# peteroh23/ModulationDetectionCNN

Hardware: AMD Instinct MI355X
Metric: I/Q frames/sec (2x128, VT-CNN2, batch=2^20) (higher is better)
Workload: dtype bf16; 1 GPU; vtcnn2-c11-bf16-n2^20; topology=vtcnn2, classes=11, frames_per_gpu=1048576, global_batch=1048576, parallelism=batch-shard x1 (no collective), outputs=softmax probabilities f32 + argmax int32, frames_per_forward_call=1048576, full=False

## Files before the change

### modulationdetectioncnn_amd/csrc/vtcnn2_bf16_sched.hip

```cpp
#include "vtcnn2_bf16_common.h"
#include "vtcnn2_sched_common.h"

#include <cmath>
#include <cstdlib>
#include <type_traits>

namespace mdc {

namespace {

constexpr int kNV = 24;

struct SchedState {
    u32x4 Wv[kNV];
    u32x4 Wa[kWFrags - kNV];
    f32x4 bias[5];
    u32x4 A1[2];
    unsigned Bf[2][2][2][4];
    f32x16 X[2];
    f32x4 rp[4];
    float rc[4];
    float tprev;
    u32x4 L0[3];
    u32x4 L1;
    unsigned cb[4];
    unsigned wr_addr, rd_addr, rc_addr, im_addr;
    int gs;
};

template <int SP, int J, int I, bool PAD = false>
__device__ __forceinline__ void sch_tap(SchedState& st, f32x4 (&acc)[5]) {
    constexpr int CT = 1 - I / 10, BB = (I / 5) % 2, OT = I % 5;
    constexpr int IDX = ((CT * 3 + J) * 2 + BB) * 5 + OT;
    const u32x4 b = u32x4{st.Bf[SP][CT][BB][0], st.Bf[SP][CT][BB][1], st.Bf[SP][CT][BB][2], st.Bf[SP][CT][BB][3]};
    if constexpr (J == 0 && I < 5) {
        if constexpr (IDX < kNV) asm volatile("v_mfma_f32_16x16x32_bf16 %0, %1, %2, %3" : "=&a"(acc[OT]) : "v"(st.Wv[IDX]), "v"(b), "a"(st.bias[OT]));
        else asm volatile("v_mfma_f32_16x16x32_bf16 %0, %1, %2, %3" : "=&a"(acc[OT]) : "a"(st.Wa[IDX - kNV]), "v"(b), "a"(st.bias[OT]));
    } else if constexpr (PAD) {
        static_assert(IDX >= kNV, "padded form written for the AGPR-resident fragments only");
        asm volatile("s_nop 1\n\tv_mfma_f32_16x16x32_bf16 %0, %1, %2, %0" : "+a"(acc[OT]) : "a"(st.Wa[IDX - kNV]), "v"(b));
    } else {
        if constexpr (IDX < kNV) asm volatile("v_mfma_f32_16x16x32_bf16 %0, %1, %2, %0" : "+a"(acc[OT]) : "v"(st.Wv[IDX]), "v"(b));
        else asm volatile("v_mfma_f32_16x16x32_bf16 %0, %1, %2, %0" : "+a"(acc[OT]) : "a"(st.Wa[IDX - kNV]), "v"(b));
    }
}
template <int SP, int U>
__device__ __forceinline__ void sch_packop(SchedState& st) {
    constexpr int CT = U >> 3, j = U & 7;
    unsigned& d = st.Bf[SP][CT][j >> 2][j & 3];
    const float lo = st.X[CT][2 * j], hi = st.X[CT][2 * j + 1];
    asm volatile("v_cvt_pk_bf16_f32 %0, %1, %2 clamp" : "=v"(d) : "v"(lo), "v"(hi));
}
template <int V12, bool FIRST, bool LAST, int ABL, bool RANGE = false>
__device__ __forceinline__ void sch_step(SchedState& st, int v, int q, unsigned short* fbase, f32x4 (&acc)[3][5], int wlo = 0) {
    constexpr int PAR = V12 & 1, PN = 1 - PAR;
    constexpr int R1 = (V12 + 1) & 3, S0 = ((V12 + 1) >> 2) % 3, SN = (S0 + 1) % 3;
    constexpr bool kLoadEven = (V12 & 3) == 1 && !LAST, kLoadOdd = (V12 & 3) == 3 && !LAST;
    constexpr int LSLOT = ((V12 >> 2) + 1) % 3;
    constexpr bool kExch = ABL != 2 && ABL != 6, kFin = ABL != 3 && ABL != 6, kC1 = ABL != 5 && ABL != 6;
    f32x4 (&a2)[5] = acc[V12 % 3];
    f32x4 (&a1)[5] = acc[(V12 + 1) % 3];
    f32x4 (&a0)[5] = acc[(V12 + 2) % 3];
    const unsigned load_addr = st.im_addr + ((v >> 2) * 16 + (kLoadEven ? 16 : 24));
    FinTmp ft;
    FinOut fo;
    constexpr int OP = (V12 + 1) & 1;
#define FIN(K) do { if (!FIRST && kFin) sch_fin_clamp<K, OP>(st, ft, fo); } while (0)
#define PREP(I) do { if (!LAST && kC1 && ABL != 11) sch_prep<R1, S0, SN, I>(st); } while (0)
#define C1M(CT) do { if (!LAST && kC1) sch_conv1_mfma<R1, S0, CT>(st); } while (0)
#define ST(W) do { if (!FIRST && kFin && (W == 0 || OP == 1)) { if (ABL == 7) { if (W == 0) asm volatile("" ::"v"(fo.o0), "v"(fo.o1)); else asm volatile("" ::"v"(fo.tt)); } else if (!RANGE || v - 1 >= wlo) sch_store<W>(fo, fbase, v - 1, q, st.gs); } } while (0)
#define WR(OT) do { if (kExch && ABL != 8) sch_part_write<PAR, OT>(st, a2[OT]); } while (0)
#define PK(N) do { if (!LAST && kC1 && ABL != 10) sch_packop<PN, N>(st); } while (0)
#define RD(R) do { if (kExch && ABL != 9) sch_red_load1<PAR, R>(st); } while (0)
#define LD() do { if (kC1 && ABL != 11) { if (kLoadEven) sch_load_even<LSLOT>(st, load_addr); else if (kLoadOdd) sch_load_odd(st, load_addr); } } while (0)
#ifdef MDC_F8_PROBE_HALF_BARRIER
    constexpr bool kHalfBarrierSkip = (V12 & 1) == 1;
#else
    constexpr bool kHalfBarrierSkip = false;
#endif
#define HANDOFF() do { \
        if (ABL == 1 || kHalfBarrierSkip) asm volatile("s_waitcnt lgkmcnt(0)" ::: "memory"); \
        else if (kExch) asm volatile("s_waitcnt lgkmcnt(0)\n\ts_barrier" ::: "memory"); \
        asm volatile("" ::"a"(a2[0]), "a"(a2[1]), "a"(a2[2]), "a"(a2[3]), "a"(a2[4])); } while (0)
    sch_wait_lds(st);
    sch_tap<PAR, 2, 0, RANGE && (V12 == 1 || V12 == 2)>(st, a2); FIN(0);
    sch_tap<PAR, 2, 1>(st, a2); FIN(1);
    sch_tap<PAR, 2, 2>(st, a2); FIN(2);
    sch_tap<PAR, 2, 3>(st, a2); FIN(3);
    sch_tap<PAR, 2, 4>(st, a2); FIN(4);
    sch_tap<PAR, 2, 5>(st, a2); FIN(5);
    sch_tap<PAR, 2, 6>(st, a2); FIN(6);
    sch_tap<PAR, 2, 7>(st, a2); FIN(7);
    sch_tap<PAR, 2, 8>(st, a2); FIN(8);
    sch_tap<PAR, 2, 9>(st, a2); FIN(9);
    sch_tap<PAR, 2, 10>(st, a2); FIN(10);
    sch_tap<PAR, 2, 11>(st, a2); FIN(11);
    sch_tap<PAR, 2, 12>(st, a2); FIN(12);
    sch_tap<PAR, 2, 13>(st, a2); FIN(13);
    sch_tap<PAR, 2, 14>(st, a2); FIN(14);
    sch_tap<PAR, 2, 15>(st, a2); FIN(15);
    sch_tap<PAR, 2, 16>(st, a2); PREP(0);
    sch_tap<PAR, 2, 17>(st, a2); PREP(1);
    sch_tap<PAR, 2, 18>(st, a2); PREP(2);
    sch_tap<PAR, 2, 19>(st, a2); PREP(3);
    C1M(0); WR(0); FIN(16); FIN(17);
    C1M(1); WR(1);
    sch_tap<PAR, 1, 0>(st, a1); ST(0);
    sch_tap<PAR, 1, 1>(st, a1); WR(2);
    sch_tap<PAR, 1, 2>(st, a1); ST(1);
    sch_tap<PAR, 1, 3>(st, a1); PK(0);
    sch_tap<PAR, 1, 4>(st, a1); WR(3);
    sch_tap<PAR, 1, 5>(st, a1); PK(1);
    sch_tap<PAR, 1, 6>(st, a1); PK(2);
    sch_tap<PAR, 1, 7>(st, a1); WR(4);
    sch_tap<PAR, 1, 8>(st, a1); PK(3);
    sch_tap<PAR, 1, 9>(st, a1); PK(4);
    sch_tap<PAR, 1, 10>(st, a1); PK(5);
    sch_tap<PAR, 1, 11>(st, a1); PK(6);
    sch_tap<PAR, 1, 12>(st, a1); PK(7);
    sch_tap<PAR, 1, 13>(st, a1); PK(8);
    sch_tap<PAR, 1, 14>(st, a1); PK(9);
    sch_tap<PAR, 1, 15>(st, a1); PK(10);
    sch_tap<PAR, 1, 16>(st, a1); PK(11);
    sch_tap<PAR, 1, 17>(st, a1); PK(12);
    sch_tap<PAR, 1, 18>(st, a1); PK(13);
    sch_tap<PAR, 1, 19>(st, a1); PK(14);
    sch_tap<PAR, 0, 0>(st, a0); PK(15);
    sch_tap<PAR, 0, 1>(st, a0);
    sch_tap<PAR, 0, 2>(st, a0);
    sch_tap<PAR, 0, 3>(st, a0);
    sch_tap<PAR, 0, 4>(st, a0);
    sch_tap<PAR, 0, 5>(st, a0);
    sch_tap<PAR, 0, 6>(st, a0); HANDOFF();
    sch_tap<PAR, 0, 7>(st, a0); RD(0);
    sch_tap<PAR, 0, 8>(st, a0); RD(1);
    sch_tap<PAR, 0, 9>(st, a0); RD(2);
    sch_tap<PAR, 0, 10>(st, a0); RD(3);
    sch_tap<PAR, 0, 11>(st, a0); RD(4);
    sch_tap<PAR, 0, 12>(st, a0); RD(5);
    sch_tap<PAR, 0, 13>(st, a0); RD(6);
    sch_tap<PAR, 0, 14>(st, a0); RD(7);
    sch_tap<PAR, 0, 15>(st, a0); LD();
    sch_tap<PAR, 0, 16>(st, a0);
    sch_tap<PAR, 0, 17>(st, a0);
    sch_tap<PAR, 0, 18>(st, a0);
    sch_tap<PAR, 0, 19>(st, a0);
    if (ABL == 10 && !LAST) asm volatile("" ::"v"(st.X[0]), "v"(st.X[1]));
#undef FIN
#undef PREP
#undef C1M
#undef ST
#undef WR
#undef PK
#undef RD
#undef LD
#undef HANDOFF
}

template <int ABL, bool U8 = false, bool RANGE = false>
__global__ __launch_bounds__(256, 1) void vt_conv_bf16_sched_kernel(const float* __restrict__ x, long n,
                                                                    const u32x4* __restrict__ wq, const u32x4* __restrict__ a1q,
                                                                    const float* __restrict__ b2, unsigned short* __restrict__ feat,
                                                                    long hop2 = 256, float scale = 0.f) {
    extern __shared__ __attribute__((aligned(16))) unsigned char smem[];
    unsigned* img = reinterpret_cast<unsigned*>(smem);
    const int tid = threadIdx.x, lane = tid & 63;
    const int q = __builtin_amdgcn_readfirstlane(tid >> 6);
// ... 17 lines not shown
    const unsigned part_lds = (unsigned)(size_t)(__attribute__((address_space(3))) unsigned char*)(smem + (size_t)2 * kSImgWords * 4);
    const unsigned img_lds = (unsigned)(size_t)(__attribute__((address_space(3))) unsigned char*)smem;
    auto entry = [](int f, int gg) { return 8 * (4 * (f >> 3) + gg) + ((f & 7) ^ (gg >> 1)); };
    const int fs = lane >> 2, gs = lane & 3;
    st.gs = gs;
    st.wr_addr = part_lds + (q * 5 * 64 + entry(nl, g)) * 16;
    st.rd_addr = part_lds + (q * 64 + entry(fs, gs)) * 16;
    st.rc_addr = part_lds + (4 * 64 + entry(fs, q)) * 16 + gs * 4;
#pragma unroll
    for (int k = 0; k < 4; ++k) { st.rp[k] = f32x4{0.f, 0.f, 0.f, 0.f}; st.rc[k] = 0.f; }
#pragma unroll
    for (int s = 0; s < 3; ++s) st.L0[s] = u32x4{0u, 0u, 0u, 0u};
    st.L1 = u32x4{0u, 0u, 0u, 0u};
    st.cb[0] = st.cb[1] = st.cb[2] = st.cb[3] = 0u;
    st.tprev = 0.f;

    for (int i = tid; i < 2 * kSImgWords; i += 256) img[i] = ((((i / kS) & 63) >= 32) && ((i % kS) & 1)) ? 0x3F803F80u : 0u;
    __syncthreads();
    const long ngroups = (n + 15) >> 4;
    long grp = blockIdx.x;
    if (grp < ngroups)
        for (int k = 0; k < 4; ++k) sch_stage_write(k, stage_decode<U8>(stage_load<U8>(k, x, n, grp * 16, tid, hop2), tid, scale), n, grp * 16, img, tid);
    __syncthreads();
    const int rng = RANGE ? (int)blockIdx.y : 0;
    const int S = 12 * rng;
    const int wlo = rng ? S + 2 : 0;

    int buf = 0;
    for (; grp < ngroups; grp += gridDim.x, buf ^= 1) {
        st.im_addr = img_lds + (buf * kSImgWords + lane * kS) * 4;
        unsigned short* fbase = feat + (grp * 16 + fs) * (long)(kW2 * kC2);
        const long gnext = RANGE ? ngroups : grp + gridDim.x;
        f32x4 acc[3][5];
        {
            const u32x4 zero = u32x4{0u, 0u, 0u, 0u};
#pragma unroll
            for (int b = 0; b < 5; ++b) {
                asm volatile("s_nop 1\n\tv_mfma_f32_16x16x32_bf16 %0, %1, %1, %2" : "=&a"(acc[0][b]) : "v"(zero), "a"(st.bias[b]));
                asm volatile("v_mfma_f32_16x16x32_bf16 %0, %1, %1, %2" : "=&a"(acc[1][b]) : "v"(zero), "a"(st.bias[b]));
            }
        }

        sch_load_even<0>(st, st.im_addr + (S >> 2) * 16);
        sch_load_odd(st, st.im_addr + (S >> 2) * 16 + 8);
        sch_wait_lds(st);
        sch_conv1_mfma<0, 0, 0>(st); sch_conv1_mfma<0, 0, 1>(st);
        asm volatile("s_nop 7\n\ts_nop 7\n\ts_nop 7\n\ts_nop 7\n\ts_nop 7\n\ts_nop 7\n\ts_nop 7\n\ts_nop 7" : "+v"(st.X[0]), "+v"(st.X[1]));
        [&]<int... N>(std::integer_sequence<int, N...>) { (sch_packop<0, N>(st), ...); }(std::make_integer_sequence<int, 16>{});
        asm volatile("s_nop 1");

        sch_step<0, true, false, ABL, RANGE>(st, S, q, fbase, acc, wlo);
        const int iters = RANGE ? (rng < 10 ? 1 : 0) : 10;
        int v = S + 1;
        typename StageRaw<U8>::type sv{};
        for (int it = 0; it < iters; ++it, v += 12) {
            if constexpr (!RANGE) {
                if (it >= 6 && gnext < ngroups) sch_stage_write(it - 6, stage_decode<U8>(sv, tid, scale), n, gnext * 16, img + (buf ^ 1) * kSImgWords, tid);
                if (it >= 5 && it < 9 && gnext < ngroups) sv = stage_load<U8>(it - 5, x, n, gnext * 16, tid, hop2);
            }
            sch_step<1, false, false, ABL, RANGE>(st, v + 0, q, fbase, acc, wlo);
            sch_step<2, false, false, ABL, RANGE>(st, v + 1, q, fbase, acc, wlo);
            sch_step<3, false, false, ABL, RANGE>(st, v + 2, q, fbase, acc, wlo);
            sch_step<4, false, false, ABL, RANGE>(st, v + 3, q, fbase, acc, wlo);
            sch_step<5, false, false, ABL, RANGE>(st, v + 4, q, fbase, acc, wlo);
            sch_step<6, false, false, ABL, RANGE>(st, v + 5, q, fbase, acc, wlo);
            sch_step<7, false, false, ABL, RANGE>(st, v + 6, q, fbase, acc, wlo);
            sch_step<8, false, false, ABL, RANGE>(st, v + 7, q, fbase, acc, wlo);
            sch_step<9, false, false, ABL, RANGE>(st, v + 8, q, fbase, acc, wlo);
            sch_step<10, false, false, ABL, RANGE>(st, v + 9, q, fbase, acc, wlo);
            sch_step<11, false, false, ABL, RANGE>(st, v + 10, q, fbase, acc, wlo);
            sch_step<0, false, false, ABL, RANGE>(st, v + 11, q, fbase, acc, wlo);
        }
        const int vt = RANGE ? v : 121;
        sch_step<1, false, false, ABL, RANGE>(st, vt, q, fbase, acc, wlo);
        if constexpr (RANGE) {
            if (rng < 10) {
                FinOut fo;
                sch_wait_lds(st);
                sch_fin_all_clamp<1>(st, fo);
                sch_store<0>(fo, fbase, vt, q, st.gs);
                sch_store<1>(fo, fbase, vt, q, st.gs);
                asm volatile("s_nop 7\n\ts_nop 7" ::"a"(acc[0][0]), "a"(acc[1][0]), "a"(acc[2][0]));
                __syncthreads();
                continue;
            }
        }
        sch_step<2, false, false, ABL, RANGE>(st, 122, q, fbase, acc, wlo);
        sch_step<3, false, false, ABL, RANGE>(st, 123, q, fbase, acc, wlo);
        sch_step<4, false, false, ABL, RANGE>(st, 124, q, fbase, acc, wlo);
        sch_step<5, false, false, ABL, RANGE>(st, 125, q, fbase, acc, wlo);
        sch_step<6, false, false, ABL, RANGE>(st, 126, q, fbase, acc, wlo);
        sch_step<7, false, false, ABL, RANGE>(st, 127, q, fbase, acc, wlo);
        sch_step<8, false, false, ABL, RANGE>(st, 128, q, fbase, acc, wlo);
        sch_step<9, false, true, ABL, RANGE>(st, 129, q, fbase, acc, wlo);
        auto finish_store = [&](auto odd, int w) {
            FinOut fo;
            sch_wait_lds(st);
            sch_fin_all_clamp<decltype(odd)::value>(st, fo);
            sch_store<0>(fo, fbase, w, q, st.gs);
            if constexpr (decltype(odd)::value) sch_store<1>(fo, fbase, w, q, st.gs);
        };
        using Even = std::integral_constant<int, 0>;
        using Odd = std::integral_constant<int, 1>;
        finish_store(Odd{}, 129);
        asm volatile("s_nop 7\n\ts_nop 7");
        sch_part_write<0, 0>(st, acc[1][0]); sch_part_write<0, 1>(st, acc[1][1]); sch_part_write<0, 2>(st, acc[1][2]);
        sch_part_write<0, 3>(st, acc[1][3]); sch_part_write<0, 4>(st, acc[1][4]);
        asm volatile("s_waitcnt lgkmcnt(0)\n\ts_barrier" ::: "memory");
        sch_red_load<0>(st);
        asm volatile("" ::"a"(acc[1][0]), "a"(acc[1][1]), "a"(acc[1][2]), "a"(acc[1][3]), "a"(acc[1][4]));
        finish_store(Even{}, 130);
        sch_part_write<1, 0>(st, acc[2][0]); sch_part_write<1, 1>(st, acc[2][1]); sch_part_write<1, 2>(st, acc[2][2]);
        sch_part_write<1, 3>(st, acc[2][3]); sch_part_write<1, 4>(st, acc[2][4]);
        asm volatile("s_waitcnt lgkmcnt(0)\n\ts_barrier" ::: "memory");
        sch_red_load<1>(st);
        asm volatile("" ::"a"(acc[2][0]), "a"(acc[2][1]), "a"(acc[2][2]), "a"(acc[2][3]), "a"(acc[2][4]));
        finish_store(Odd{}, 131);
        __syncthreads();
    }
}

}

int vtcnn2_bf16_pack_sched(mdc_model* m) {
    const float* k1 = m->hk[0].data();
    const float* b1 = m->hb[0].data();
    const float* k2 = m->hk[1].data();
    int rc;
    std::vector<unsigned short> wq((size_t)4 * kWFrags * 64 * 8);
    for (int q = 0; q < 4; ++q)
        for (int ct = 0; ct < 2; ++ct)
            for (int j = 0; j < 3; ++j)
                for (int bb = 0; bb < 2; ++bb)
// ... 20 lines not shown
                }
                if (khalf == 0) {
                    d[0] = th[0]; d[1] = th[1]; d[2] = th[0]; d[3] = th[1]; d[4] = th[2]; d[6] = th[2];
                } else {
                    const unsigned short bh = f2bf(b1[ch] * sc);
                    d[0] = tl[0]; d[1] = tl[1]; d[2] = bh; d[3] = f2bf(b1[ch] * sc - bf2f(bh)); d[4] = tl[2];
                }
            }
    return upload(m, 7, a1.data(), a1.size() * 2);
}

int vtcnn2_bf16_conv_sched(const mdc_model* m, const float* x, int64_t n, void* feat, hipStream_t s, long hop2, float scale) {
    const long ngroups = (n + 15) / 16;
    const unsigned grid = (unsigned)(ngroups < 256 ? ngroups : 256);
#define MDC_LAUNCH_SCHED_V(U, R, GRID) do { \
    MDC_HIP(hipFuncSetAttribute(reinterpret_cast<const void*>(vt_conv_bf16_sched_kernel<0, U, R>), hipFuncAttributeMaxDynamicSharedMemorySize, (int)kSchedLds)); \
    hipLaunchKernelGGL((vt_conv_bf16_sched_kernel<0, U, R>), GRID, dim3(256), kSchedLds, s, x, (long)n, \
                       static_cast<const u32x4*>(m->d_pack[6]), static_cast<const u32x4*>(m->d_pack[7]), \
                       static_cast<const float*>(m->d_pack[2]), static_cast<unsigned short*>(feat), hop2 > 0 ? hop2 : 256L, scale); \
    MDC_HIP(hipGetLastError()); return MDC_OK; } while (0)
    if (n <= kConvRangeFrames) {
        if (hop2 > 0) MDC_LAUNCH_SCHED_V(true, true, dim3((unsigned)ngroups, 11));
        else MDC_LAUNCH_SCHED_V(false, true, dim3((unsigned)ngroups, 11));
    }
    if (hop2 > 0) MDC_LAUNCH_SCHED_V(true, false, dim3(grid));
#undef MDC_LAUNCH_SCHED_V
#define MDC_LAUNCH_SCHED(A) do { \
    MDC_HIP(hipFuncSetAttribute(reinterpret_cast<const void*>(vt_conv_bf16_sched_kernel<A>), hipFuncAttributeMaxDynamicSharedMemorySize, (int)kSchedLds)); \
    hipLaunchKernelGGL(vt_conv_bf16_sched_kernel<A>, dim3(grid), dim3(256), kSchedLds, s, x, (long)n, \
                       static_cast<const u32x4*>(m->d_pack[6]), static_cast<const u32x4*>(m->d_pack[7]), \
                       static_cast<const float*>(m->d_pack[2]), static_cast<unsigned short*>(feat), 256L, 0.f); } while (0)
#ifdef MDC_ABLATIONS
    static const int abl = getenv("MDC_ABLATE_S") ? atoi(getenv("MDC_ABLATE_S")) : 0;
    switch (abl) { case 1: MDC_LAUNCH_SCHED(1); break; case 2: MDC_LAUNCH_SCHED(2); break; case 3: MDC_LAUNCH_SCHED(3); break;
                   case 5: MDC_LAUNCH_SCHED(5); break; case 6: MDC_LAUNCH_SCHED(6); break; case 7: MDC_LAUNCH_SCHED(7); break;
                   case 8: MDC_LAUNCH_SCHED(8); break; case 9: MDC_LAUNCH_SCHED(9); break; case 10: MDC_LAUNCH_SCHED(10); break;
                   case 11: MDC_LAUNCH_SCHED(11); break; default: MDC_LAUNCH_SCHED(0); }
#else
    MDC_LAUNCH_SCHED(0);
#endif
#undef MDC_LAUNCH_SCHED
    MDC_HIP(hipGetLastError());
    return MDC_OK;
}

}
```

### modulationdetectioncnn_amd/csrc/vtcnn2_sched_common.h

```cpp
#pragma once
#include "vtcnn2_bf16_common.h"

#include <type_traits>
#include <utility>

namespace mdc {

namespace {

constexpr int kS = 140;
constexpr int kSImgWords = 64 * kS;
constexpr long kConvRangeFrames = 1024;
constexpr size_t kSchedLds = (size_t)2 * kSImgWords * 4 + (size_t)2 * kPartFloats * 4;

using f32x16 = __attribute__((ext_vector_type(16))) float;

template <int SLOT, class S>
__device__ __forceinline__ void sch_load_even(S& st, unsigned entry_addr) {
    asm volatile("ds_read_b128 %0, %1" : "=v"(st.L0[SLOT]) : "v"(entry_addr) : "memory");
}
template <class S>
__device__ __forceinline__ void sch_load_odd(S& st, unsigned entry_addr) {
    asm volatile("ds_read2_b64 %0, %1 offset0:0 offset1:1" : "=v"(st.L1) : "v"(entry_addr) : "memory");
}
// ... 18 lines not shown
template <int PB, int OT, class S>
__device__ __forceinline__ void sch_part_write(S& st, const f32x4& a) {
    asm volatile("ds_write_b128 %0, %1 offset:%2" ::"v"(st.wr_addr), "a"(a), "i"(PB * kPartFloats * 4 + OT * 1024) : "memory");
}
template <int PB, int R, class S>
__device__ __forceinline__ void sch_red_load1(S& st) {
    constexpr int K = R >> 1;
    if constexpr ((R & 1) == 0) asm volatile("ds_read_b128 %0, %1 offset:%2" : "=v"(st.rp[K]) : "v"(st.rd_addr), "i"(PB * kPartFloats * 4 + K * 5120) : "memory");
    else asm volatile("ds_read_b32 %0, %1 offset:%2" : "=v"(st.rc[K]) : "v"(st.rc_addr), "i"(PB * kPartFloats * 4 + K * 5120) : "memory");
}
template <int PB, class S>
__device__ __forceinline__ void sch_red_load(S& st) {
    sch_red_load1<PB, 0>(st); sch_red_load1<PB, 1>(st); sch_red_load1<PB, 2>(st); sch_red_load1<PB, 3>(st);
    sch_red_load1<PB, 4>(st); sch_red_load1<PB, 5>(st); sch_red_load1<PB, 6>(st); sch_red_load1<PB, 7>(st);
}
template <class S>
__device__ __forceinline__ void sch_wait_lds(S& st) {
    asm volatile("s_waitcnt lgkmcnt(0)"
                 : "+v"(st.rp[0]), "+v"(st.rp[1]), "+v"(st.rp[2]), "+v"(st.rp[3]), "+v"(st.rc[0]), "+v"(st.rc[1]), "+v"(st.rc[2]),
                   "+v"(st.rc[3]), "+v"(st.L0[0]), "+v"(st.L0[1]), "+v"(st.L0[2]), "+v"(st.L1)
                 :: "memory");
}
struct FinOut { unsigned o0, o1, tt; };
struct FinTmp { float s[4], u[4], a, b, t; };
constexpr int kFeatShift = 32;

template <int K, int ODD, class S>
__device__ __forceinline__ void sch_fin_clamp(S& st, FinTmp& f, FinOut& out) {
    if constexpr (K < 4) asm volatile("v_add_f32 %0, %1, %2" : "=v"(f.s[K]) : "v"(st.rp[0][K]), "v"(st.rp[1][K]));
    else if constexpr (K < 8) asm volatile("v_add_f32 %0, %1, %2" : "=v"(f.u[K - 4]) : "v"(st.rp[2][K - 4]), "v"(st.rp[3][K - 4]));
    else if constexpr (K < 12) asm volatile("v_add_f32 %0, %0, %1" : "+v"(f.s[K - 8]) : "v"(f.u[K - 8]));
    else if constexpr (K == 12) asm volatile("v_cvt_pk_bf16_f32 %0, %1, %2 clamp" : "=v"(out.o0) : "v"(f.s[0]), "v"(f.s[1]));
    else if constexpr (K == 13) asm volatile("v_cvt_pk_bf16_f32 %0, %1, %2 clamp" : "=v"(out.o1) : "v"(f.s[2]), "v"(f.s[3]));
    else if constexpr (K == 14) asm volatile("v_add_f32 %0, %1, %2" : "=v"(f.a) : "v"(st.rc[0]), "v"(st.rc[1]));
    else if constexpr (K == 15) asm volatile("v_add_f32 %0, %1, %2" : "=v"(f.b) : "v"(st.rc[2]), "v"(st.rc[3]));
    else if constexpr (K == 16) {
// ... 20 lines not shown
    if (frame0 + i >= n) v = make_float4(0.f, 0.f, 0.f, 0.f);
    const int h = l >> 5, m = l & 31;
    const float xs[4] = {v.x, v.y, v.z, v.w};
#pragma unroll
    for (int e = 0; e < 2; ++e) {
        const float a = xs[2 * e], b = xs[2 * e + 1];
        const unsigned hi = pack2(a, b);
        const float ah = __uint_as_float(hi << 16), bh = __uint_as_float(hi & 0xFFFF0000u);
        const unsigned lo = pack2(a - ah, b - bh);
        unsigned* d = im + (i + 16 * h) * kS + 2 * (2 * m + 1 + e);
        *reinterpret_cast<u32x2*>(d) = u32x2{hi, lo};
        d[32 * kS] = hi;
    }
}


}

}
```

Measured before the change: 40.67 million frames/s.

## Overlap group epilogue with next group prologue and interleave staging into MFMA gaps

The tail of each frame group (steps 130/131 partial exchange, reduction and stores) is folded into the next group's first step. It uses an extra LDS partial buffer and cross-group finalize/store with a deferred last store. Next-group input staging (bf16 hi/lo split and LDS writes) is broken into single instructions and placed into gaps between MFMAs in the last iterations, rather than done as bulk code. This removes the serialized drain and barrier between groups and hides staging ALU work, at the cost of more LDS, more complex control and register pressure.

```diff
diff --git a/modulationdetectioncnn_amd/csrc/vtcnn2_bf16_sched.hip b/modulationdetectioncnn_amd/csrc/vtcnn2_bf16_sched.hip
--- a/modulationdetectioncnn_amd/csrc/vtcnn2_bf16_sched.hip
+++ b/modulationdetectioncnn_amd/csrc/vtcnn2_bf16_sched.hip
@@ -9,6 +9,7 @@
 
 namespace {
 
+constexpr size_t kSchedLdsX = kSchedLds + (size_t)2 * kPartBytes;
 constexpr int kNV = 24;
 
 struct SchedState {
@@ -26,14 +27,20 @@
     unsigned cb[4];
     unsigned wr_addr, rd_addr, rc_addr, im_addr;
     int gs;
+    StageGap sg;
 };
 
-template <int SP, int J, int I, bool PAD = false>
+struct PartX { f32x4 rp[4]; float rc[4]; float tprev; };
+
+template <int SP, int J, int I, bool PAD = false, bool OPEN = false>
 __device__ __forceinline__ void sch_tap(SchedState& st, f32x4 (&acc)[5]) {
     constexpr int CT = 1 - I / 10, BB = (I / 5) % 2, OT = I % 5;
     constexpr int IDX = ((CT * 3 + J) * 2 + BB) * 5 + OT;
     const u32x4 b = u32x4{st.Bf[SP][CT][BB][0], st.Bf[SP][CT][BB][1], st.Bf[SP][CT][BB][2], st.Bf[SP][CT][BB][3]};
-    if constexpr (J == 0 && I < 5) {
+    if constexpr (OPEN && J == 2 && I == 0) {
+        static_assert(IDX >= kNV, "the opening MFMAs of taps 1 and 2 use AGPR-resident fragments");
+        asm volatile("s_nop 1\n\tv_mfma_f32_16x16x32_bf16 %0, %1, %2, %3" : "=&a"(acc[OT]) : "a"(st.Wa[IDX - kNV]), "v"(b), "a"(st.bias[OT]));
+    } else if constexpr ((J == 0 || OPEN) && I < 5) {
         if constexpr (IDX < kNV) asm volatile("v_mfma_f32_16x16x32_bf16 %0, %1, %2, %3" : "=&a"(acc[OT]) : "v"(st.Wv[IDX]), "v"(b), "a"(st.bias[OT]));
         else asm volatile("v_mfma_f32_16x16x32_bf16 %0, %1, %2, %3" : "=&a"(acc[OT]) : "a"(st.Wa[IDX - kNV]), "v"(b), "a"(st.bias[OT]));
     } else if constexpr (PAD) {
@@ -51,10 +58,11 @@
     const float lo = st.X[CT][2 * j], hi = st.X[CT][2 * j + 1];
     asm volatile("v_cvt_pk_bf16_f32 %0, %1, %2 clamp" : "=v"(d) : "v"(lo), "v"(hi));
 }
-template <int V12, bool FIRST, bool LAST, int ABL, bool RANGE = false>
-__device__ __forceinline__ void sch_step(SchedState& st, int v, int q, unsigned short* fbase, f32x4 (&acc)[3][5], int wlo = 0) {
+template <int V12, bool FIRST, bool LAST, int ABL, bool RANGE = false, bool XG = false, bool XLD = false, int STG = 0>
+__device__ __forceinline__ void sch_step(SchedState& st, int v, int q, unsigned short* fbase, f32x4 (&acc)[3][5], int wlo = 0, unsigned xoff = 0, PartX* px = nullptr) {
     constexpr int PAR = V12 & 1, PN = 1 - PAR;
-    constexpr int R1 = (V12 + 1) & 3, S0 = ((V12 + 1) >> 2) % 3, SN = (S0 + 1) % 3;
+    constexpr bool kX1 = LAST && !RANGE && ABL != 13 && ABL != 15;
+    constexpr int R1 = LAST ? 0 : (V12 + 1) & 3, S0 = LAST ? 0 : ((V12 + 1) >> 2) % 3, SN = (S0 + 1) % 3;
     constexpr bool kLoadEven = (V12 & 3) == 1 && !LAST, kLoadOdd = (V12 & 3) == 3 && !LAST;
     constexpr int LSLOT = ((V12 >> 2) + 1) % 3;
     constexpr bool kExch = ABL != 2 && ABL != 6, kFin = ABL != 3 && ABL != 6, kC1 = ABL != 5 && ABL != 6;
@@ -65,14 +73,19 @@
     FinTmp ft;
     FinOut fo;
     constexpr int OP = (V12 + 1) & 1;
-#define FIN(K) do { if (!FIRST && kFin) sch_fin_clamp<K, OP>(st, ft, fo); } while (0)
+    static_assert(!(XG && (RANGE || !FIRST)) && !(XLD && V12 != 8) && !(STG && (LAST || FIRST)), "cross-group roles");
+    static_assert(!LAST || (PAR == 1 && V12 % 3 == 0), "step 129: Bf[0] is free for the next group, a1 = acc[1] = output 130");
+#define FIN(K) do { if ((!FIRST || XG) && kFin) sch_fin_clamp<K, OP>(st, ft, fo); } while (0)
 #define PREP(I) do { if (!LAST && kC1 && ABL != 11) sch_prep<R1, S0, SN, I>(st); } while (0)
-#define C1M(CT) do { if (!LAST && kC1) sch_conv1_mfma<R1, S0, CT>(st); } while (0)
-#define ST(W) do { if (!FIRST && kFin && (W == 0 || OP == 1)) { if (ABL == 7) { if (W == 0) asm volatile("" ::"v"(fo.o0), "v"(fo.o1)); else asm volatile("" ::"v"(fo.tt)); } else if (!RANGE || v - 1 >= wlo) sch_store<W>(fo, fbase, v - 1, q, st.gs); } } while (0)
+#define C1M(CT) do { if ((!LAST || kX1) && kC1) sch_conv1_mfma<R1, S0, CT>(st); } while (0)
+#define ST(W) do { if ((!FIRST || XG) && kFin && (W == 0 || OP == 1)) { if (ABL == 7) { if (W == 0) asm volatile("" ::"v"(fo.o0), "v"(fo.o1)); else asm volatile("" ::"v"(fo.tt)); } else if (RANGE ? v - 1 >= wlo : (!XG || wlo != 0)) sch_store<W>(fo, fbase, v - 1, q, st.gs); } } while (0)
 #define WR(OT) do { if (kExch && ABL != 8) sch_part_write<PAR, OT>(st, a2[OT]); } while (0)
-#define PK(N) do { if (!LAST && kC1 && ABL != 10) sch_packop<PN, N>(st); } while (0)
+#define WRX(OT) do { if (LAST && !RANGE && kExch && ABL != 8) sch_part_write_at<0, OT>(wrx, a1[OT]); } while (0)
+#define RDX(R) do { if (LAST && !RANGE && kExch && ABL != 9) sch_red_load1_at<0, R>(*px, rdx, rcx); } while (0)
+#define PK(N) do { if ((!LAST || kX1) && kC1 && ABL != 10) sch_packop<PN, N>(st); } while (0)
 #define RD(R) do { if (kExch && ABL != 9) sch_red_load1<PAR, R>(st); } while (0)
-#define LD() do { if (kC1 && ABL != 11) { if (kLoadEven) sch_load_even<LSLOT>(st, load_addr); else if (kLoadOdd) sch_load_odd(st, load_addr); } } while (0)
+#define LD() do { if (kC1 && ABL != 11) { if (kX1) sch_load_odd(st, xim); else if (XLD) sch_load_even<0>(st, xim); else if (kLoadEven) sch_load_even<LSLOT>(st, load_addr); else if (kLoadOdd) sch_load_odd(st, load_addr); } } while (0)
+#define SG(N) do { if constexpr (STG == 1) sch_stage_op<N>(st.sg); else if constexpr (STG == 2) sch_stage_op<9 + N>(st.sg); else if constexpr (STG == 3 && (N == 5 || N == 6)) sch_stage_op<13 + N>(st.sg); } while (0)
 #ifdef MDC_F8_PROBE_HALF_BARRIER
     constexpr bool kHalfBarrierSkip = (V12 & 1) == 1;
 #else
@@ -81,13 +94,14 @@
 #define HANDOFF() do { \
         if (ABL == 1 || kHalfBarrierSkip) asm volatile("s_waitcnt lgkmcnt(0)" ::: "memory"); \
         else if (kExch) asm volatile("s_waitcnt lgkmcnt(0)\n\ts_barrier" ::: "memory"); \
-        asm volatile("" ::"a"(a2[0]), "a"(a2[1]), "a"(a2[2]), "a"(a2[3]), "a"(a2[4])); } while (0)
+        asm volatile("" ::"a"(a2[0]), "a"(a2[1]), "a"(a2[2]), "a"(a2[3]), "a"(a2[4])); \
+        if (LAST && !RANGE) asm volatile("" ::"a"(a1[0]), "a"(a1[1]), "a"(a1[2]), "a"(a1[3]), "a"(a1[4])); } while (0)
     sch_wait_lds(st);
-    sch_tap<PAR, 2, 0, RANGE && (V12 == 1 || V12 == 2)>(st, a2); FIN(0);
-    sch_tap<PAR, 2, 1>(st, a2); FIN(1);
-    sch_tap<PAR, 2, 2>(st, a2); FIN(2);
-    sch_tap<PAR, 2, 3>(st, a2); FIN(3);
-    sch_tap<PAR, 2, 4>(st, a2); FIN(4);
+    sch_tap<PAR, 2, 0, RANGE && (V12 == 1 || V12 == 2), FIRST>(st, a2); FIN(0);
+    sch_tap<PAR, 2, 1, false, FIRST>(st, a2); FIN(1);
+    sch_tap<PAR, 2, 2, false, FIRST>(st, a2); FIN(2);
+    sch_tap<PAR, 2, 3, false, FIRST>(st, a2); FIN(3);
+    sch_tap<PAR, 2, 4, false, FIRST>(st, a2); FIN(4);
     sch_tap<PAR, 2, 5>(st, a2); FIN(5);
     sch_tap<PAR, 2, 6>(st, a2); FIN(6);
     sch_tap<PAR, 2, 7>(st, a2); FIN(7);
@@ -99,17 +113,18 @@
     sch_tap<PAR, 2, 13>(st, a2); FIN(13);
     sch_tap<PAR, 2, 14>(st, a2); FIN(14);
     sch_tap<PAR, 2, 15>(st, a2); FIN(15);
-    sch_tap<PAR, 2, 16>(st, a2); PREP(0);
-    sch_tap<PAR, 2, 17>(st, a2); PREP(1);
-    sch_tap<PAR, 2, 18>(st, a2); PREP(2);
-    sch_tap<PAR, 2, 19>(st, a2); PREP(3);
+    unsigned wrx = 0, xim = 0, rdx = 0, rcx = 0;
+    sch_tap<PAR, 2, 16>(st, a2); PREP(0); if constexpr (LAST && !RANGE) wrx = st.wr_addr + 2 * kPartBytes;
+    sch_tap<PAR, 2, 17>(st, a2); PREP(1); if constexpr (kX1) xim = st.im_addr + xoff + 8;
+    sch_tap<PAR, 2, 18>(st, a2); PREP(2); if constexpr (LAST && !RANGE) rdx = st.rd_addr + 2 * kPartBytes;
+    sch_tap<PAR, 2, 19>(st, a2); PREP(3); if constexpr (LAST && !RANGE) rcx = st.rc_addr + 2 * kPartBytes;
     C1M(0); WR(0); FIN(16); FIN(17);
     C1M(1); WR(1);
-    sch_tap<PAR, 1, 0>(st, a1); ST(0);
-    sch_tap<PAR, 1, 1>(st, a1); WR(2);
-    sch_tap<PAR, 1, 2>(st, a1); ST(1);
-    sch_tap<PAR, 1, 3>(st, a1); PK(0);
-    sch_tap<PAR, 1, 4>(st, a1); WR(3);
+    sch_tap<PAR, 1, 0, false, FIRST>(st, a1); ST(0);
+    sch_tap<PAR, 1, 1, false, FIRST>(st, a1); WR(2);
+    sch_tap<PAR, 1, 2, false, FIRST>(st, a1); ST(1);
+    sch_tap<PAR, 1, 3, false, FIRST>(st, a1); PK(0);
+    sch_tap<PAR, 1, 4, false, FIRST>(st, a1); WR(3);
     sch_tap<PAR, 1, 5>(st, a1); PK(1);
     sch_tap<PAR, 1, 6>(st, a1); PK(2);
     sch_tap<PAR, 1, 7>(st, a1); WR(4);
@@ -126,11 +141,11 @@
     sch_tap<PAR, 1, 18>(st, a1); PK(13);
     sch_tap<PAR, 1, 19>(st, a1); PK(14);
     sch_tap<PAR, 0, 0>(st, a0); PK(15);
-    sch_tap<PAR, 0, 1>(st, a0);
-    sch_tap<PAR, 0, 2>(st, a0);
-    sch_tap<PAR, 0, 3>(st, a0);
-    sch_tap<PAR, 0, 4>(st, a0);
-    sch_tap<PAR, 0, 5>(st, a0);
+    sch_tap<PAR, 0, 1>(st, a0); WRX(0); SG(0); if constexpr (XLD) xim = st.im_addr + xoff;
+    sch_tap<PAR, 0, 2>(st, a0); WRX(1); SG(1);
+    sch_tap<PAR, 0, 3>(st, a0); WRX(2); SG(2);
+    sch_tap<PAR, 0, 4>(st, a0); WRX(3); SG(3);
+    sch_tap<PAR, 0, 5>(st, a0); WRX(4); SG(4);
     sch_tap<PAR, 0, 6>(st, a0); HANDOFF();
     sch_tap<PAR, 0, 7>(st, a0); RD(0);
     sch_tap<PAR, 0, 8>(st, a0); RD(1);
@@ -141,16 +156,19 @@
     sch_tap<PAR, 0, 13>(st, a0); RD(6);
     sch_tap<PAR, 0, 14>(st, a0); RD(7);
     sch_tap<PAR, 0, 15>(st, a0); LD();
-    sch_tap<PAR, 0, 16>(st, a0);
-    sch_tap<PAR, 0, 17>(st, a0);
-    sch_tap<PAR, 0, 18>(st, a0);
-    sch_tap<PAR, 0, 19>(st, a0);
-    if (ABL == 10 && !LAST) asm volatile("" ::"v"(st.X[0]), "v"(st.X[1]));
+    sch_tap<PAR, 0, 16>(st, a0); SG(5); RDX(0); RDX(1);
+    sch_tap<PAR, 0, 17>(st, a0); SG(6); RDX(2); RDX(3);
+    sch_tap<PAR, 0, 18>(st, a0); SG(7); RDX(4); RDX(5);
+    sch_tap<PAR, 0, 19>(st, a0); SG(8); RDX(6); RDX(7);
+    if (ABL == 10 && (!LAST || kX1)) asm volatile("" ::"v"(st.X[0]), "v"(st.X[1]));
 #undef FIN
 #undef PREP
 #undef C1M
 #undef ST
 #undef WR
+#undef WRX
+#undef RDX
+#undef SG
 #undef PK
 #undef RD
 #undef LD
@@ -198,33 +216,25 @@
     st.L1 = u32x4{0u, 0u, 0u, 0u};
     st.cb[0] = st.cb[1] = st.cb[2] = st.cb[3] = 0u;
     st.tprev = 0.f;
+    st.sg = StageGap{{0.f, 0.f, 0.f, 0.f}, {0u, 0u}, {0u, 0u}, 0u, 0u};
 
     for (int i = tid; i < 2 * kSImgWords; i += 256) img[i] = ((((i / kS) & 63) >= 32) && ((i % kS) & 1)) ? 0x3F803F80u : 0u;
     __syncthreads();
     const long ngroups = (n + 15) >> 4;
     long grp = blockIdx.x;
+    constexpr bool kNoDrain = ABL == 12 || ABL == 15, kNoStage = ABL == 14 || ABL == 15;
     if (grp < ngroups)
-        for (int k = 0; k < 4; ++k) sch_stage_write(k, stage_decode<U8>(stage_load<U8>(k, x, n, grp * 16, tid, hop2), tid, scale), n, grp * 16, img, tid);
+        for (int k = 0; k < 4; ++k) {
+            const float4 v4 = stage_decode<U8>(stage_load<U8>(k, x, n, grp * 16, tid, hop2), tid, scale);
+            sch_stage_write(k, v4, n, grp * 16, img, tid);
+            if constexpr (kNoStage) sch_stage_write(k, v4, n, grp * 16, img + kSImgWords, tid);
+        }
     __syncthreads();
     const int rng = RANGE ? (int)blockIdx.y : 0;
     const int S = 12 * rng;
     const int wlo = rng ? S + 2 : 0;
 
-    int buf = 0;
-    for (; grp < ngroups; grp += gridDim.x, buf ^= 1) {
-        st.im_addr = img_lds + (buf * kSImgWords + lane * kS) * 4;
-        unsigned short* fbase = feat + (grp * 16 + fs) * (long)(kW2 * kC2);
-        const long gnext = RANGE ? ngroups : grp + gridDim.x;
-        f32x4 acc[3][5];
-        {
-            const u32x4 zero = u32x4{0u, 0u, 0u, 0u};
-#pragma unroll
-            for (int b = 0; b < 5; ++b) {
-                asm volatile("s_nop 1\n\tv_mfma_f32_16x16x32_bf16 %0, %1, %1, %2" : "=&a"(acc[0][b]) : "v"(zero), "a"(st.bias[b]));
-                asm volatile("v_mfma_f32_16x16x32_bf16 %0, %1, %1, %2" : "=&a"(acc[1][b]) : "v"(zero), "a"(st.bias[b]));
-            }
-        }
-
+    auto prologue = [&]() {
         sch_load_even<0>(st, st.im_addr + (S >> 2) * 16);
         sch_load_odd(st, st.im_addr + (S >> 2) * 16 + 8);
         sch_wait_lds(st);
@@ -232,19 +242,39 @@
         asm volatile("s_nop 7\n\ts_nop 7\n\ts_nop 7\n\ts_nop 7\n\ts_nop 7\n\ts_nop 7\n\ts_nop 7\n\ts_nop 7" : "+v"(st.X[0]), "+v"(st.X[1]));
         [&]<int... N>(std::integer_sequence<int, N...>) { (sch_packop<0, N>(st), ...); }(std::make_integer_sequence<int, 16>{});
         asm volatile("s_nop 1");
-
-        sch_step<0, true, false, ABL, RANGE>(st, S, q, fbase, acc, wlo);
+    };
+    st.im_addr = img_lds + lane * kS * 4;
+    if constexpr (!RANGE) prologue();
+
+    const unsigned sw_addr = img_lds + ((q + 16 * (lane >> 5)) * kS + 2 * (2 * (lane & 31) + 1)) * 4;
+    const long gstride = (long)gridDim.x * 16 * (kW2 * kC2);
+    int has_prev = 0;
+    int buf = 0;
+    for (; grp < ngroups; grp += gridDim.x, buf ^= 1) {
+        st.im_addr = img_lds + (buf * kSImgWords + lane * kS) * 4;
+        const unsigned xoff = (buf ? -1 : 1) * (kSImgWords * 4);
+        unsigned short* fbase = feat + (grp * 16 + fs) * (long)(kW2 * kC2);
+        const long gnext = RANGE ? ngroups : grp + gridDim.x;
+        f32x4 acc[3][5];
+        if constexpr (RANGE) prologue();
+        if constexpr (RANGE) sch_step<0, true, false, ABL, true>(st, S, q, fbase, acc, wlo);
+        else sch_step<0, true, false, ABL, false, true>(st, 132, q, fbase - gstride, acc, has_prev);
         const int iters = RANGE ? (rng < 10 ? 1 : 0) : 10;
         int v = S + 1;
+        if constexpr (RANGE) asm volatile("" : "+s"(v));
         typename StageRaw<U8>::type sv{};
-        for (int it = 0; it < iters; ++it, v += 12) {
-            if constexpr (!RANGE) {
-                if (it >= 6 && gnext < ngroups) sch_stage_write(it - 6, stage_decode<U8>(sv, tid, scale), n, gnext * 16, img + (buf ^ 1) * kSImgWords, tid);
-                if (it >= 5 && it < 9 && gnext < ngroups) sv = stage_load<U8>(it - 5, x, n, gnext * 16, tid, hop2);
+        auto steps12 = [&](auto sge, int ldq) {
+            constexpr bool SGE = decltype(sge)::value;
+            sch_step<1, false, false, ABL, RANGE, false, false, SGE ? 1 : 0>(st, v + 0, q, fbase, acc, wlo);
+            sch_step<2, false, false, ABL, RANGE, false, false, SGE ? 2 : 0>(st, v + 1, q, fbase, acc, wlo);
+            sch_step<3, false, false, ABL, RANGE, false, false, SGE ? 3 : 0>(st, v + 2, q, fbase, acc, wlo);
+            if constexpr (!RANGE && !U8) {
+                if (ldq >= 0) {
+                    const long f = gnext * 16 + q + 4 * ldq;
+                    const float4 r = reinterpret_cast<const float4*>(x + (f < n ? f : n - 1) * kFrameFloats)[lane];
+                    st.sg.x[0] = r.x; st.sg.x[1] = r.y; st.sg.x[2] = r.z; st.sg.x[3] = r.w;
+                }
             }
-            sch_step<1, false, false, ABL, RANGE>(st, v + 0, q, fbase, acc, wlo);
-            sch_step<2, false, false, ABL, RANGE>(st, v + 1, q, fbase, acc, wlo);
-            sch_step<3, false, false, ABL, RANGE>(st, v + 2, q, fbase, acc, wlo);
             sch_step<4, false, false, ABL, RANGE>(st, v + 3, q, fbase, acc, wlo);
             sch_step<5, false, false, ABL, RANGE>(st, v + 4, q, fbase, acc, wlo);
             sch_step<6, false, false, ABL, RANGE>(st, v + 5, q, fbase, acc, wlo);
@@ -254,6 +284,22 @@
             sch_step<10, false, false, ABL, RANGE>(st, v + 9, q, fbase, acc, wlo);
             sch_step<11, false, false, ABL, RANGE>(st, v + 10, q, fbase, acc, wlo);
             sch_step<0, false, false, ABL, RANGE>(st, v + 11, q, fbase, acc, wlo);
+        };
+        constexpr bool kGapStage = !RANGE && !U8 && !kNoStage;
+        const int plain = kGapStage ? 6 : iters;
+        for (int it = 0; it < plain; ++it, v += 12) {
+            if constexpr (!RANGE && !kNoStage && U8) {
+                if (it >= 6 && gnext < ngroups) sch_stage_write(it - 6, stage_decode<U8>(sv, tid, scale), n, gnext * 16, img + (buf ^ 1) * kSImgWords, tid);
+                if (it >= 5 && it < 9 && gnext < ngroups) sv = stage_load<U8>(it - 5, x, n, gnext * 16, tid, hop2);
+            }
+            steps12(std::false_type{}, kGapStage && it == 5 && gnext < ngroups ? 0 : -1);
+        }
+        if constexpr (kGapStage) {
+            for (int it = 6; it < 10; ++it, v += 12) {
+                st.sg.addr = sw_addr + (buf ^ 1) * (kSImgWords * 4) + (it - 6) * (4 * kS * 4);
+                st.sg.mask = gnext * 16 + q + 4 * (it - 6) < n ? 0xFFFFFFFFu : 0u;
+                steps12(std::true_type{}, it < 9 && gnext < ngroups ? it - 5 : -1);
+            }
         }
         const int vt = RANGE ? v : 121;
         sch_step<1, false, false, ABL, RANGE>(st, vt, q, fbase, acc, wlo);
@@ -275,32 +321,75 @@
         sch_step<5, false, false, ABL, RANGE>(st, 125, q, fbase, acc, wlo);
         sch_step<6, false, false, ABL, RANGE>(st, 126, q, fbase, acc, wlo);
         sch_step<7, false, false, ABL, RANGE>(st, 127, q, fbase, acc, wlo);
-        sch_step<8, false, false, ABL, RANGE>(st, 128, q, fbase, acc, wlo);
-        sch_step<9, false, true, ABL, RANGE>(st, 129, q, fbase, acc, wlo);
-        auto finish_store = [&](auto odd, int w) {
+        sch_step<8, false, false, ABL, RANGE, false, !RANGE>(st, 128, q, fbase, acc, wlo, xoff);
+        PartX px;
+        sch_step<9, false, true, ABL, RANGE>(st, 129, q, fbase, acc, wlo, xoff, &px);
+        has_prev = 1;
+        if constexpr (RANGE) {
+            auto finish_store = [&](auto odd, int w) {
+                FinOut fo;
+                sch_wait_lds(st);
+                sch_fin_all_clamp<decltype(odd)::value>(st, fo);
+                sch_store<0>(fo, fbase, w, q, st.gs);
+                if constexpr (decltype(odd)::value) sch_store<1>(fo, fbase, w, q, st.gs);
+            };
+            using Even = std::integral_constant<int, 0>;
+            using Odd = std::integral_constant<int, 1>;
+            finish_store(Odd{}, 129);
+            asm volatile("s_nop 7\n\ts_nop 7");
+            sch_part_write<0, 0>(st, acc[1][0]); sch_part_write<0, 1>(st, acc[1][1]); sch_part_write<0, 2>(st, acc[1][2]);
+            sch_part_write<0, 3>(st, acc[1][3]); sch_part_write<0, 4>(st, acc[1][4]);
+            asm volatile("s_waitcnt lgkmcnt(0)\n\ts_barrier" ::: "memory");
+            sch_red_load<0>(st);
+            asm volatile("" ::"a"(acc[1][0]), "a"(acc[1][1]), "a"(acc[1][2]), "a"(acc[1][3]), "a"(acc[1][4]));
+            finish_store(Even{}, 130);
+            sch_part_write<1, 0>(st, acc[2][0]); sch_part_write<1, 1>(st, acc[2][1]); sch_part_write<1, 2>(st, acc[2][2]);
+            sch_part_write<1, 3>(st, acc[2][3]); sch_part_write<1, 4>(st, acc[2][4]);
+            asm volatile("s_waitcnt lgkmcnt(0)\n\ts_barrier" ::: "memory");
+            sch_red_load<1>(st);
+            asm volatile("" ::"a"(acc[2][0]), "a"(acc[2][1]), "a"(acc[2][2]), "a"(acc[2][3]), "a"(acc[2][4]));
+            finish_store(Odd{}, 131);
+            continue;
+        }
+        if constexpr (kNoDrain) {
+            asm volatile("" ::"a"(acc[2][0]), "a"(acc[2][1]), "a"(acc[2][2]), "a"(acc[2][3]), "a"(acc[2][4]));
+            continue;
+        }
+        {
+            FinTmp ft, ftx;
+            FinOut fo, fox;
+            using Head = std::integer_sequence<int, 0, 1, 2, 3, 4, 5, 6, 7, 14, 15>;
+            using Rest = std::integer_sequence<int, 8, 9, 10, 11, 12, 13, 16, 17>;
+            auto fin = [&]<int... K>(std::integer_sequence<int, K...>) { (sch_fin_clamp<K, 1>(st, ft, fo), ...); };
+            auto finx = [&]<int... K>(std::integer_sequence<int, K...>) { (sch_fin_clamp<K, 0>(px, ftx, fox), ...); };
+            sch_wait_lds_but<8>(st);
+            fin(Head{});
+            asm volatile("s_nop 7\n\ts_nop 7");
+            const unsigned wr2 = st.wr_addr + 2 * kPartBytes, rd2 = st.rd_addr + 2 * kPartBytes, rc2 = st.rc_addr + 2 * kPartBytes;
+            sch_part_write_at<1, 0>(wr2, acc[2][0]); sch_part_write_at<1, 1>(wr2, acc[2][1]); sch_part_write_at<1, 2>(wr2, acc[2][2]);
+            sch_part_write_at<1, 3>(wr2, acc[2][3]); sch_part_write_at<1, 4>(wr2, acc[2][4]);
+            fin(Rest{});
+            asm volatile("s_waitcnt lgkmcnt(5)" : "+v"(px.rp[0]), "+v"(px.rp[1]), "+v"(px.rp[2]), "+v"(px.rp[3]), "+v"(px.rc[0]), "+v"(px.rc[1]), "+v"(px.rc[2]), "+v"(px.rc[3]) :: "memory");
+            finx(Head{});
+            finx(Rest{});
+            st.tprev = px.tprev;
+            sch_store<0>(fo, fbase, 129, q, st.gs);
+            sch_store<1>(fo, fbase, 129, q, st.gs);
+            sch_store<0>(fox, fbase, 130, q, st.gs);
+            asm volatile("s_waitcnt lgkmcnt(0)\n\ts_barrier" ::: "memory");
+            asm volatile("" ::"a"(acc[2][0]), "a"(acc[2][1]), "a"(acc[2][2]), "a"(acc[2][3]), "a"(acc[2][4]));
+            sch_red_load_at<1>(st, rd2, rc2);
+        }
+    }
+    if constexpr (!RANGE) {
+        if (has_prev) {
             FinOut fo;
             sch_wait_lds(st);
-            sch_fin_all_clamp<decltype(odd)::value>(st, fo);
-            sch_store<0>(fo, fbase, w, q, st.gs);
-            if constexpr (decltype(odd)::value) sch_store<1>(fo, fbase, w, q, st.gs);
-        };
-        using Even = std::integral_constant<int, 0>;
-        using Odd = std::integral_constant<int, 1>;
-        finish_store(Odd{}, 129);
-        asm volatile("s_nop 7\n\ts_nop 7");
-        sch_part_write<0, 0>(st, acc[1][0]); sch_part_write<0, 1>(st, acc[1][1]); sch_part_write<0, 2>(st, acc[1][2]);
-        sch_part_write<0, 3>(st, acc[1][3]); sch_part_write<0, 4>(st, acc[1][4]);
-        asm volatile("s_waitcnt lgkmcnt(0)\n\ts_barrier" ::: "memory");
-        sch_red_load<0>(st);
-        asm volatile("" ::"a"(acc[1][0]), "a"(acc[1][1]), "a"(acc[1][2]), "a"(acc[1][3]), "a"(acc[1][4]));
-        finish_store(Even{}, 130);
-        sch_part_write<1, 0>(st, acc[2][0]); sch_part_write<1, 1>(st, acc[2][1]); sch_part_write<1, 2>(st, acc[2][2]);
-        sch_part_write<1, 3>(st, acc[2][3]); sch_part_write<1, 4>(st, acc[2][4]);
-        asm volatile("s_waitcnt lgkmcnt(0)\n\ts_barrier" ::: "memory");
-        sch_red_load<1>(st);
-        asm volatile("" ::"a"(acc[2][0]), "a"(acc[2][1]), "a"(acc[2][2]), "a"(acc[2][3]), "a"(acc[2][4]));
-        finish_store(Odd{}, 131);
-        __syncthreads();
+            sch_fin_all_clamp<1>(st, fo);
+            unsigned short* flast = feat + ((grp - gridDim.x) * 16 + fs) * (long)(kW2 * kC2);
+            sch_store<0>(fo, flast, 131, q, st.gs);
+            sch_store<1>(fo, flast, 131, q, st.gs);
+        }
     }
 }
 
@@ -351,8 +440,8 @@
     const long ngroups = (n + 15) / 16;
     const unsigned grid = (unsigned)(ngroups < 256 ? ngroups : 256);
 #define MDC_LAUNCH_SCHED_V(U, R, GRID) do { \
-    MDC_HIP(hipFuncSetAttribute(reinterpret_cast<const void*>(vt_conv_bf16_sched_kernel<0, U, R>), hipFuncAttributeMaxDynamicSharedMemorySize, (int)kSchedLds)); \
-    hipLaunchKernelGGL((vt_conv_bf16_sched_kernel<0, U, R>), GRID, dim3(256), kSchedLds, s, x, (long)n, \
+    MDC_HIP(hipFuncSetAttribute(reinterpret_cast<const void*>(vt_conv_bf16_sched_kernel<0, U, R>), hipFuncAttributeMaxDynamicSharedMemorySize, (int)kSchedLdsX)); \
+    hipLaunchKernelGGL((vt_conv_bf16_sched_kernel<0, U, R>), GRID, dim3(256), kSchedLdsX, s, x, (long)n, \
                        static_cast<const u32x4*>(m->d_pack[6]), static_cast<const u32x4*>(m->d_pack[7]), \
                        static_cast<const float*>(m->d_pack[2]), static_cast<unsigned short*>(feat), hop2 > 0 ? hop2 : 256L, scale); \
     MDC_HIP(hipGetLastError()); return MDC_OK; } while (0)
@@ -363,8 +452,8 @@
     if (hop2 > 0) MDC_LAUNCH_SCHED_V(true, false, dim3(grid));
 #undef MDC_LAUNCH_SCHED_V
 #define MDC_LAUNCH_SCHED(A) do { \
-    MDC_HIP(hipFuncSetAttribute(reinterpret_cast<const void*>(vt_conv_bf16_sched_kernel<A>), hipFuncAttributeMaxDynamicSharedMemorySize, (int)kSchedLds)); \
-    hipLaunchKernelGGL(vt_conv_bf16_sched_kernel<A>, dim3(grid), dim3(256), kSchedLds, s, x, (long)n, \
+    MDC_HIP(hipFuncSetAttribute(reinterpret_cast<const void*>(vt_conv_bf16_sched_kernel<A>), hipFuncAttributeMaxDynamicSharedMemorySize, (int)kSchedLdsX)); \
+    hipLaunchKernelGGL(vt_conv_bf16_sched_kernel<A>, dim3(grid), dim3(256), kSchedLdsX, s, x, (long)n, \
                        static_cast<const u32x4*>(m->d_pack[6]), static_cast<const u32x4*>(m->d_pack[7]), \
                        static_cast<const float*>(m->d_pack[2]), static_cast<unsigned short*>(feat), 256L, 0.f); } while (0)
 #ifdef MDC_ABLATIONS
@@ -372,7 +461,8 @@
     switch (abl) { case 1: MDC_LAUNCH_SCHED(1); break; case 2: MDC_LAUNCH_SCHED(2); break; case 3: MDC_LAUNCH_SCHED(3); break;
                    case 5: MDC_LAUNCH_SCHED(5); break; case 6: MDC_LAUNCH_SCHED(6); break; case 7: MDC_LAUNCH_SCHED(7); break;
                    case 8: MDC_LAUNCH_SCHED(8); break; case 9: MDC_LAUNCH_SCHED(9); break; case 10: MDC_LAUNCH_SCHED(10); break;
-                   case 11: MDC_LAUNCH_SCHED(11); break; default: MDC_LAUNCH_SCHED(0); }
+                   case 11: MDC_LAUNCH_SCHED(11); break; case 12: MDC_LAUNCH_SCHED(12); break; case 13: MDC_LAUNCH_SCHED(13); break;
+                   case 14: MDC_LAUNCH_SCHED(14); break; case 15: MDC_LAUNCH_SCHED(15); break; default: MDC_LAUNCH_SCHED(0); }
 #else
     MDC_LAUNCH_SCHED(0);
 #endif
diff --git a/modulationdetectioncnn_amd/csrc/vtcnn2_sched_common.h b/modulationdetectioncnn_amd/csrc/vtcnn2_sched_common.h
--- a/modulationdetectioncnn_amd/csrc/vtcnn2_sched_common.h
+++ b/modulationdetectioncnn_amd/csrc/vtcnn2_sched_common.h
@@ -56,12 +56,45 @@
     sch_red_load1<PB, 0>(st); sch_red_load1<PB, 1>(st); sch_red_load1<PB, 2>(st); sch_red_load1<PB, 3>(st);
     sch_red_load1<PB, 4>(st); sch_red_load1<PB, 5>(st); sch_red_load1<PB, 6>(st); sch_red_load1<PB, 7>(st);
 }
+constexpr unsigned kPartBytes = kPartFloats * 4;
+template <int PB, int OT>
+__device__ __forceinline__ void sch_part_write_at(unsigned wr, const f32x4& a) {
+    asm volatile("ds_write_b128 %0, %1 offset:%2" ::"v"(wr), "a"(a), "i"(PB * kPartFloats * 4 + OT * 1024) : "memory");
+}
+template <int PB, int R, class S>
+__device__ __forceinline__ void sch_red_load1_at(S& st, unsigned rd, unsigned rc) {
+    constexpr int K = R >> 1;
+    if constexpr ((R & 1) == 0) asm volatile("ds_read_b128 %0, %1 offset:%2" : "=v"(st.rp[K]) : "v"(rd), "i"(PB * kPartFloats * 4 + K * 5120) : "memory");
+    else asm volatile("ds_read_b32 %0, %1 offset:%2" : "=v"(st.rc[K]) : "v"(rc), "i"(PB * kPartFloats * 4 + K * 5120) : "memory");
+}
+template <int PB, class S>
+__device__ __forceinline__ void sch_red_load_at(S& st, unsigned rd, unsigned rc) {
+    [&]<int... R>(std::integer_sequence<int, R...>) { (sch_red_load1_at<PB, R>(st, rd, rc), ...); }(std::make_integer_sequence<int, 8>{});
+}
+template <unsigned OFF>
+__device__ __forceinline__ unsigned sch_addr_plus(unsigned a) {
+    unsigned r;
+    asm volatile("v_add_u32 %0, %1, %2" : "=v"(r) : "i"(OFF), "v"(a));
+    return r;
+}
+__device__ __forceinline__ unsigned sch_addr_plus_s(unsigned a, unsigned uniform_off) {
+    unsigned r;
+    asm volatile("v_add_u32 %0, %1, %2" : "=v"(r) : "s"(uniform_off), "v"(a));
+    return r;
+}
 template <class S>
 __device__ __forceinline__ void sch_wait_lds(S& st) {
     asm volatile("s_waitcnt lgkmcnt(0)"
                  : "+v"(st.rp[0]), "+v"(st.rp[1]), "+v"(st.rp[2]), "+v"(st.rp[3]), "+v"(st.rc[0]), "+v"(st.rc[1]), "+v"(st.rc[2]),
                    "+v"(st.rc[3]), "+v"(st.L0[0]), "+v"(st.L0[1]), "+v"(st.L0[2]), "+v"(st.L1)
                  :: "memory");
+}
+template <int N, class S>
+__device__ __forceinline__ void sch_wait_lds_but(S& st) {
+    asm volatile("s_waitcnt lgkmcnt(%12)"
+                 : "+v"(st.rp[0]), "+v"(st.rp[1]), "+v"(st.rp[2]), "+v"(st.rp[3]), "+v"(st.rc[0]), "+v"(st.rc[1]), "+v"(st.rc[2]),
+                   "+v"(st.rc[3]), "+v"(st.L0[0]), "+v"(st.L0[1]), "+v"(st.L0[2]), "+v"(st.L1)
+                 : "i"(N) : "memory");
 }
 struct FinOut { unsigned o0, o1, tt; };
 struct FinTmp { float s[4], u[4], a, b, t; };
@@ -112,6 +145,26 @@
     }
 }
 
+struct StageGap { float x[4]; unsigned hi[2], lo[2]; unsigned addr, mask; };
+template <int N>
+__device__ __forceinline__ void sch_stage_op(StageGap& g) {
+    constexpr unsigned kUp = 32 * kS * 4;
+    if constexpr (N == 0) asm volatile("v_cvt_pk_bf16_f32 %0, %1, %2" : "=v"(g.hi[0]) : "v"(g.x[0]), "v"(g.x[1]));
+    else if constexpr (N == 1) asm volatile("v_cvt_pk_bf16_f32 %0, %1, %2" : "=v"(g.hi[1]) : "v"(g.x[2]), "v"(g.x[3]));
+    else if constexpr (N == 2 || N == 6) asm volatile("v_lshlrev_b32 %0, 16, %1" : "=v"(g.lo[0]) : "v"(g.hi[N == 6]));
+    else if constexpr (N == 3 || N == 7) asm volatile("v_and_b32 %0, 0xffff0000, %1" : "=v"(g.lo[1]) : "v"(g.hi[N == 7]));
+    else if constexpr (N == 4 || N == 5) asm volatile("v_sub_f32 %0, %0, %1" : "+v"(g.x[N - 4]) : "v"(g.lo[N - 4]));
+    else if constexpr (N == 8 || N == 9) asm volatile("v_sub_f32 %0, %0, %1" : "+v"(g.x[N - 6]) : "v"(g.lo[N - 8]));
+    else if constexpr (N == 10) asm volatile("v_cvt_pk_bf16_f32 %0, %1, %2" : "=v"(g.lo[0]) : "v"(g.x[0]), "v"(g.x[1]));
+    else if constexpr (N == 11) asm volatile("v_cvt_pk_bf16_f32 %0, %1, %2" : "=v"(g.lo[1]) : "v"(g.x[2]), "v"(g.x[3]));
+    else if constexpr (N == 12 || N == 14) asm volatile("v_and_b32 %0, %1, %0" : "+v"(g.hi[N == 14]) : "s"(g.mask));
+    else if constexpr (N == 13 || N == 15) asm volatile("v_and_b32 %0, %1, %0" : "+v"(g.lo[N == 15]) : "s"(g.mask));
+    else if constexpr (N == 16) asm volatile("ds_write2_b32 %0, %1, %2 offset0:0 offset1:1" ::"v"(g.addr), "v"(g.hi[0]), "v"(g.lo[0]) : "memory");
+    else if constexpr (N == 17) asm volatile("ds_write_b32 %0, %1 offset:%2" ::"v"(g.addr), "v"(g.hi[0]), "i"(kUp) : "memory");
+    else if constexpr (N == 18) asm volatile("ds_write2_b32 %0, %1, %2 offset0:2 offset1:3" ::"v"(g.addr), "v"(g.hi[1]), "v"(g.lo[1]) : "memory");
+    else if constexpr (N == 19) asm volatile("ds_write_b32 %0, %1 offset:%2" ::"v"(g.addr), "v"(g.hi[1]), "i"(kUp + 8) : "memory");
+}
+
 
 }
 
```

After: 40.97 million frames/s, median of 6. About the same (+0.7%).
